# timsainb/noisereduce

Hardware: AMD Instinct MI355X
Metric: Msamples/s reduce_noise (48 kHz mono, n_fft=1024) (higher is better)
Workload: dtype f32

## Files before the change

### include/mi355gate_debug.h

```cpp
#ifndef MI355GATE_DEBUG_H
#define MI355GATE_DEBUG_H

#include "mi355gate.h"

#ifdef __cplusplus
extern "C" {
#endif

SG_API int sg_debug_dims(const sg_handle* h, int64_t dims[3]);
SG_API int sg_debug_range(const sg_handle* h, int64_t range[2]);
SG_API int sg_debug_counter(sg_handle* h, int32_t which, int64_t* value, void* stream);
SG_API int sg_debug_fetch(sg_handle* h, int32_t what, void* host, int64_t bytes, void* stream);

SG_API int sg_debug_clip_thresholds(sg_handle* h, double* host, int32_t n_noise, int32_t n_bins, void* stream);
SG_API int sg_debug_clip_batches(const sg_handle* h, int64_t* value);
SG_API int sg_debug_rows_batches(const sg_handle* h, int64_t* value);
#define SG_BWD_ROW 1
#define SG_BWD_FAST 2
#define SG_BWD_REG 3
#define SG_BWD_OLA 4
#define SG_BWD_ROWS 5
SG_API int sg_debug_backward_route(const sg_handle* h, int64_t* value);

#define SG_OPT_FORCE_UNFUSED 1
#define SG_OPT_FORCE_F64_DECIDE 3
#define SG_OPT_FORCE_NOSEAM 4
#define SG_OPT_FORCE_NOLEAN 5
#define SG_OPT_FORCE_SPLIT 6
#define SG_OPT_INJECT_HANDOFF_FAULT 7
#define SG_OPT_FORCE_NOROWGATE 10
#define SG_OPT_ROWGATE_TAP 11
#define SG_OPT_ROWGATE_SHAPE 12
#define SG_OPT_FLOOR_TEST 13
#define SG_OPT_TILE_ORDER 15
#define SG_OPT_EXACT_MATERIALISED 16
#define SG_OPT_FORCE_NOFAST 2

#define SG_STAGE_CHANNEL_MEAN 0
#define SG_STAGE_STFT_POWER 1
#define SG_STAGE_COLMAX 2
#define SG_STAGE_COLSTATS 3
#define SG_STAGE_DECIDE 4
#define SG_STAGE_STFT_MAG 5
#define SG_STAGE_NONSTAT_MASK 6
#define SG_STAGE_SMOOTH 7
#define SG_STAGE_APPLY_ISTFT 8
#define SG_STAGE_OLA 9
#define SG_STAGE_NOISE_STATS 10
#define SG_STAGE_PREP 11
// ... 29 lines not shown
```

### noisereduce_amd/_ffi.py

```python
import contextlib
import ctypes
import os
import threading
import weakref
from ctypes import (POINTER, Structure, byref, c_char_p, c_double, c_int, c_int32,
                    c_int64, c_void_p)

import numpy as np
import torch

_HERE = os.path.dirname(os.path.abspath(__file__))
LIB_PATH = os.path.join(_HERE, "libmi355gate.so")

SG_F32, SG_F64, SG_I16, SG_I32 = 0, 1, 2, 3
SG_VARIANT_S, SG_VARIANT_T = 0, 1
SG_E_INVALID, SG_E_UNSUPPORTED, SG_E_HIP, SG_E_NOMEM, SG_E_STATE, SG_E_HANDOFF = -1, -2, -3, -4, -5, -6
SG_N_STAGES = 27
SG_N_STAGES_ALL = 29
SG_OPT_FORCE_F64_DECIDE = 3
SG_OPT_FORCE_NOSEAM = 4
SG_OPT_FORCE_NOLEAN = 5
SG_OPT_FORCE_SPLIT = 6
SG_OPT_INJECT_HANDOFF_FAULT = 7
SG_OPT_FAST_INTEGER = 8
SG_OPT_FORCE_EXACT = 9
SG_OPT_FORCE_NOROWGATE = 10
SG_OPT_ROWGATE_TAP = 11
SG_OPT_ROWGATE_SHAPE = 12
SG_OPT_FLOOR_TEST = 13
SG_OPT_TILE_ORDER = 15
SG_OPT_EXACT_MATERIALISED = 16
SG_OPT_FORCE_UNFUSED = 1
SG_OPT_FORCE_NOFAST = 2
SG_BWD_ROW, SG_BWD_FAST, SG_BWD_REG, SG_BWD_OLA, SG_BWD_ROWS = 1, 2, 3, 4, 5

_TORCH_DTYPES = {torch.float32: SG_F32, torch.float64: SG_F64, torch.int16: SG_I16,
                 torch.int32: SG_I32}


class HandoffTimeout(RuntimeError):
    """SG_E_HANDOFF: a bounded inter-workgroup wait of a fused kernel timed out (the device was preempted for
    about a second); the outputs of the calls enqueued since the last check are invalid and must be re-run."""


class SgParams(Structure):
    _fields_ = [
# ... 64 lines not shown
                                  c_int64, c_int64, c_int64, c_int64, c_int32, c_int64, c_int64,
                                  c_void_p]),
    "sg_filter_padded": (c_int, [c_void_p, c_void_p, c_int, c_void_p, c_int, c_int64, c_int64,
                                 c_int64, c_int64, c_void_p]),
    "sg_process_batch": (c_int, [c_void_p, c_void_p, c_int, c_int64, c_int64, c_int64, c_void_p,
                                 c_int64, c_int64, c_int64, c_void_p, c_int, c_int64, c_void_p,
                                 c_void_p]),
    "sg_process_batch_backward": (c_int, [c_void_p, c_void_p, c_int, c_int64, c_int64, c_int64,
                                          c_void_p, c_void_p, c_int64, c_void_p]),
    "sg_process_rows": (c_int, [c_void_p, c_void_p, c_int, c_int64, c_int64, c_int64, c_void_p, c_void_p, c_int64,
                                c_int64, c_int64, c_void_p, c_void_p, c_int, c_int64, c_void_p, c_void_p]),
    "sg_process_rows_backward": (c_int, [c_void_p, c_void_p, c_int, c_int64, c_int64, c_int64, c_void_p, c_void_p,
                                         c_void_p, c_int64, c_void_p]),
    "sg_debug_rows_batches": (c_int, [c_void_p, POINTER(c_int64)]),
    "sg_debug_backward_route": (c_int, [c_void_p, POINTER(c_int64)]),
    "sg_stft": (c_int, [c_void_p, c_void_p, c_int, c_int64, c_int64, c_int64, c_void_p, c_void_p]),
    "sg_clips_workspace_bytes": (c_int, [c_void_p, c_void_p, c_int32, c_void_p, c_int64, POINTER(c_int64)]),
    "sg_process_clips": (c_int, [c_void_p, c_void_p, c_int, c_void_p, c_int, c_void_p, c_int32, c_void_p, c_int64,
                                 c_void_p, c_int, c_int64, c_void_p]),
    "sg_debug_clip_thresholds": (c_int, [c_void_p, POINTER(c_double), c_int32, c_int32, c_void_p]),
    "sg_debug_clip_batches": (c_int, [c_void_p, POINTER(c_int64)]),
    "sg_stream_create": (c_int, [c_void_p, c_int32, c_int32, c_int64, POINTER(c_void_p)]),
    "sg_stream_destroy": (c_int, [c_void_p]),
    "sg_stream_set_threshold": (c_int, [c_void_p, c_void_p, c_int32, c_void_p, c_int32, c_void_p]),
    "sg_stream_push": (c_int, [c_void_p, c_void_p, c_int, c_void_p, c_int, c_void_p, c_int32, c_void_p]),
    "sg_stream_reset": (c_int, [c_void_p, c_void_p, c_int32, c_void_p]),
    "sg_stream_emitted": (c_int, [c_void_p, c_int64, POINTER(c_int64)]),
    "sg_stream_counters": (c_int, [c_void_p, c_int32, POINTER(c_int64), POINTER(c_int64)]),
    "sg_stream_create_nonstationary": (c_int, [c_void_p, c_int32, c_int32, c_int64, c_int32, POINTER(c_void_p)]),
    "sg_stream_state_bytes": (c_int, [c_void_p, c_int32, c_int32, c_int64, c_int32, POINTER(c_int64)]),
# ... 651 lines not shown
```

### noisereduce_amd/csrc/api.hip

```cpp
#include <hip/hip_runtime.h>
#include <dlfcn.h>

#include <algorithm>
#include <cmath>
#include <cstdarg>
#include <cstdio>
#include <cstring>
#include <map>
#include <mutex>
#include <string>
#include <vector>

#include "../../include/mi355gate_debug.h"
#pragma clang fp contract(on)
#include "kernels.hpp"
#include "fused.hpp"
#include "czt.hpp"
#include "mixed.hpp"
#include "onepass.hpp"
#include "rowgate.hpp"
#include "rowbwd.hpp"
#include "fast512.hpp"
#include "onepass512.hpp"
#include "fast256.hpp"
// ... 90 lines not shown
  unsigned inject_fault = 0;
  unsigned lose_now = 0;
  unsigned ticket_base = 0;
  unsigned epoch = 0;
  bool fast_integer = false;
  bool force_exact = false;
  bool exact_materialised = false;
  DevBuf norm64;
  unsigned need_era = 0;
  DevBuf xP, xraw, xM, xtmp, xseg;
  bool force_split = false;
  int rowgate_mode = 0;
  int64_t n_floor_lazy = 0, n_floor_apriori = 0;
  int tile_order = 0;
  int n_cu = 0;
  int floor_test = 0;
  int rg_shape = 16;
  bool rg_tap = false;
  bool dbg_rg = false;
  int dbg_bwd_route = 0;
  DevBuf rg_count;
  bool dbg_xbits = false;
  int dbg_trows = 16, dbg_tstep = 16, dbg_twords = 0, dbg_txw = 9;
  int64_t dbg_tf0 = 0;
  int dbg_ntt = 0;
  int big_M = 0;
  int big_czt = 0;
  DevBuf big_twM, big_tw2, big_ch, big_bh, big_W, big_W2;
  int czt_M = 0;
  bool mr_ok = false;
// ... 1815 lines not shown
}

static int handoff_next_epoch(sg_handle* h, hipStream_t st) {
  if (++h->epoch == 0) {
    if (h->xbits.p) HIPCHK(h, hipMemsetAsync(h->xbits.p, 0, h->xbits.bytes, st));
    if (h->xpart.p) HIPCHK(h, hipMemsetAsync(h->xpart.p, 0, h->xpart.bytes, st));
    h->epoch = 1;
    if (h->err_host) h->err_host[1] = 0u;
  }
  return SG_OK;
}

static int handoff_prepare(sg_handle* h, hipStream_t st) {
  {
    bool fresh = false;
    int rc = ensure_zeroed(h, h->xticket, 64, st, &fresh);
    if (rc) return rc;
    if (fresh) h->ticket_base = 0;
  }
  if (!h->err_host) {
    HIPCHK(h, hipHostMalloc((void**)&h->err_host, 64, hipHostMallocMapped));
    *h->err_host = 0u;
    h->err_host[1] = 0u;
    HIPCHK(h, hipHostGetDevicePointer((void**)&h->err_dev, h->err_host, 0));
  }
  if (*h->err_host != 0u) {
    const unsigned e = *h->err_host;
    *h->err_host = 0u;
    FAIL(h, SG_E_HANDOFF, "a tile hand-off of an EARLIER call on this handle timed out (code %u): that call's output "
                          "is invalid (call sg_check_errors after a call to learn about it in time)", e);
  }
  h->lose_now = 0;
  if (h->inject_fault) {
// ... 157 lines not shown
  P.ticket = (unsigned*)h->xticket.p;
  P.epoch = h->epoch;
  P.err = h->err_dev;
  P.ticket_base = h->ticket_base;
  const bool persist = lazy && h->tile_order == 0 && !(h->lose_now & 3u) && ub * ntt >= 2;
  if (persist && h->n_cu == 0) {
    int dev = 0, cus = 0;
    HIPCHK(h, hipGetDevice(&dev));
    HIPCHK(h, hipDeviceGetAttribute(&cus, hipDeviceAttributeMultiprocessorCount, dev));
    h->n_cu = cus > 0 ? cus : 256;
  }
  static const int pg_per_cu = [] { const char* e = getenv("SG_ONEPASS_WG_PER_CU"); int v = e ? atoi(e) : 3; return v >= 1 && v <= 3 ? v : 3; }();
#if OP_MAX_ITERS == 1
  const unsigned pgrid = persist ? (unsigned)(ub * ntt) : 0u;
#else
  const unsigned pgrid = persist ? (unsigned)std::min<int64_t>(ub * ntt, (int64_t)pg_per_cu * h->n_cu) : 0u;
#endif
  P.total_tiles = (unsigned)(ub * ntt);
  if (h->tile_order == 1) P.ticket_base = 0xffffffffu;
  else h->ticket_base += (unsigned)(ub * ntt) + (OP_MAX_ITERS == 1 ? 0u : pgrid);
  P.nf = h->p.n_grad_freq; P.nt = h->p.n_grad_time;
  P.prop = (float)h->p.prop_decrease;
  P.inv_ktot = 1.0f / (float)h->ktot;
#if OP_WHO
  if (!g_who_dev) HIPCHK(h, hipMalloc((void**)&g_who_dev, 4096 * 16));
  HIPCHK(h, hipMemsetAsync(g_who_dev, 0, 4096 * 16, st));
  P.who = g_who_dev;
#endif
#if OP_TRACE
  {
    static unsigned* tr = nullptr;
    static size_t tr_slots = 0;
    const size_t slots = (size_t)ub * ntt * 4;
    if (!tr || tr_slots < slots) {
      HIPCHK(h, hipMalloc((void**)&tr, slots * 64));
// ... 24 lines not shown
          fprintf(stderr, "[OP_TRACE] completed waves %.0f; average shader cycles per wave and phase:", w);
          double tot = 0;
          for (int k = 0; k < 14; ++k) { fprintf(stderr, " %d:%.0f", k, sum[k] / (w > 0 ? w : 1)); tot += sum[k] / (w > 0 ? w : 1); }
          fprintf(stderr, "  sum %.0f  longest wave %.0f\n", tot, mx);
        });
      }
    }
    HIPCHK(h, hipMemsetAsync(tr, 0, slots * 64, st));
    P.trace = tr;
    g_trace_dev = tr; g_trace_tiles = (size_t)ub * ntt; g_trace_ntt = (int)ntt;
  }
#endif
  {
    ProfScope ps(h, SG_STAGE_ONEPASS, st);
    const size_t lds = (size_t)(fast::FN + WAVES * fast::WAVE_CX_H) * sizeof(fast::cf) + (1024 + T2_FLOATS) * sizeof(float) +
                       256 * 8 + 514 * 8 + 192 * 8 + 32 + (prop ? 528 : 0);
    auto go = [&](auto kern) -> hipError_t {
      hipError_t e = set_lds(reinterpret_cast<const void*>(kern), lds);
      if (e != hipSuccess) return e;
      hipLaunchKernelGGL(kern, dim3(persist ? pgrid : (unsigned)(ub * ntt)), dim3(WAVES * 64), lds, st, P);
      return hipGetLastError();
    };
    if (persist && prop) HIPCHK(h, go(fast::k_gate_onepass<WAVES, true, false, false, true>));
    else if (persist) HIPCHK(h, go(fast::k_gate_onepass<WAVES, false, false, false, true>));
    else if (h->lose_now & 3u) HIPCHK(h, go(fast::k_gate_onepass<WAVES, false, true>));
    else if (prop) HIPCHK(h, go(fast::k_gate_onepass<WAVES, true>));
    else HIPCHK(h, go(fast::k_gate_onepass<WAVES, false>));
  }
  if (lazy) {
    ProfScope ps(h, SG_STAGE_STFT_MAX, st);
    const int wpr = (g.F + 63) / 64;
    HIPCHK(h, launch_bits_any<0>(h, vx, g, ub, tc,
                             (unsigned long long*)h->pmax.p, (unsigned long long*)h->bits.p, wpr, st));
    if ((rc = handoff_next_epoch(h, st))) return rc;
    P.epoch = h->epoch;
    P.ticket = (unsigned*)h->xticket.p + 8;
    P.ticket_base = 0;
    const size_t lds = (size_t)(fast::FN + WAVES * fast::WAVE_CX_H) * sizeof(fast::cf) + (1024 + T2_FLOATS) * sizeof(float) +
                       256 * 8 + 514 * 8 + 192 * 8 + 32 + (prop ? 528 : 0);
    auto redo = [&](auto kern) -> hipError_t {
      hipError_t e = set_lds(reinterpret_cast<const void*>(kern), lds);
      if (e != hipSuccess) return e;
      hipLaunchKernelGGL(kern, dim3((unsigned)(ub * ntt)), dim3(WAVES * 64), lds, st, P);
      return hipGetLastError();
    };
    if (prop) HIPCHK(h, redo(fast::k_gate_onepass<WAVES, true, false, true>));
    else HIPCHK(h, redo(fast::k_gate_onepass<WAVES, false, false, true>));
    HIPCHK(h, hipGetLastError());
  }
  h->dbg_xbits = true;
  h->dbg_trows = 16; h->dbg_tstep = 16; h->dbg_twords = fast::OP_TILE_WORDS; h->dbg_txw = fast::OP_XW;
  h->dbg_tf0 = A.h_begin - 3;
  h->dbg_ntt = (int)ntt;
  h->dbg_db = std::max<int64_t>(0, A.h_begin - 3 - NF);
// ... 819 lines not shown
    case SG_OPT_FORCE_NOROWGATE:
      if (value < 0 || value > 2) FAIL(h, SG_E_INVALID, "SG_OPT_FORCE_NOROWGATE: 0 (auto), 1 (never) or 2 (always)");
      h->rowgate_mode = (int)value;
      return SG_OK;
    case SG_OPT_ROWGATE_TAP: h->rg_tap = value != 0; return SG_OK;
    case SG_OPT_ROWGATE_SHAPE:
      if (value != 8 && value != 16) FAIL(h, SG_E_INVALID, "SG_OPT_ROWGATE_SHAPE: 8 or 16 waves");
      h->rg_shape = (int)value;
      return SG_OK;
    case SG_OPT_INJECT_HANDOFF_FAULT: h->inject_fault = (unsigned)value & 63u; return SG_OK;
    case SG_OPT_TILE_ORDER:
      if (value < 0 || value > 2) FAIL(h, SG_E_INVALID, "SG_OPT_TILE_ORDER: 0 (persistent workgroups), 1 (block index) or 2 (one ticket per workgroup)");
      h->tile_order = (int)value;
      return SG_OK;
    case SG_OPT_EXACT_MATERIALISED: h->exact_materialised = value != 0; return SG_OK;
    case SG_OPT_FLOOR_TEST:
      if (value < 0 || value > 2) FAIL(h, SG_E_INVALID, "SG_OPT_FLOOR_TEST: 0 (predicted), 1 (a priori) or 2 (in the gate kernel)");
      h->floor_test = (int)value;
      return SG_OK;
  }
  FAIL(h, SG_E_INVALID, "sg_set_option: unknown option %d", option);
}

extern "C" int sg_get_option(const sg_handle* h, int32_t option, int64_t* value) {
  if (!h || !value) return SG_E_INVALID;
  switch (option) {
    case SG_OPT_FORCE_UNFUSED: *value = h->force_unfused; return SG_OK;
    case SG_OPT_FORCE_NOFAST: *value = h->force_nofast; return SG_OK;
    case SG_OPT_FORCE_F64_DECIDE: *value = h->force_f64_decide; return SG_OK;
    case SG_OPT_FORCE_NOSEAM: *value = h->force_noseam; return SG_OK;
    case SG_OPT_FORCE_NOLEAN: *value = h->force_nolean; return SG_OK;
    case SG_OPT_FORCE_SPLIT: *value = h->force_split; return SG_OK;
    case SG_OPT_FAST_INTEGER: *value = h->fast_integer; return SG_OK;
    case SG_OPT_FORCE_EXACT: *value = h->force_exact; return SG_OK;
    case SG_OPT_FORCE_NOROWGATE: *value = h->rowgate_mode; return SG_OK;
    case SG_OPT_ROWGATE_TAP: *value = h->rg_tap; return SG_OK;
    case SG_OPT_ROWGATE_SHAPE: *value = h->rg_shape; return SG_OK;
    case SG_OPT_INJECT_HANDOFF_FAULT: *value = h->inject_fault; return SG_OK;
    case SG_OPT_TILE_ORDER: *value = h->tile_order; return SG_OK;
    case SG_OPT_EXACT_MATERIALISED: *value = h->exact_materialised; return SG_OK;
    case SG_OPT_FLOOR_TEST: *value = h->floor_test; return SG_OK;
  }
  return SG_E_INVALID;
}

extern "C" int sg_profile_enable(sg_handle* h, int32_t on) {
  if (!h) return SG_E_INVALID;
  h->prof_on = on != 0;
  return SG_OK;
}

extern "C" int sg_profile_select(sg_handle* h, int64_t stage_mask) {
  if (!h) return SG_E_INVALID;
  h->prof_mask = stage_mask == 0 ? ~0ull : (uint64_t)stage_mask;
  return SG_OK;
// ... 51 lines not shown
  if (!h || !dims) return SG_E_INVALID;
  dims[0] = h->dbg_units; dims[1] = h->dbg_T; dims[2] = h->FS;
  return SG_OK;
}

extern "C" int sg_debug_range(const sg_handle* h, int64_t range[2]) {
  if (!h || !range) return SG_E_INVALID;
  range[0] = h->dbg_db; range[1] = h->dbg_de;
  return SG_OK;
}

extern "C" int sg_debug_counter(sg_handle* h, int32_t which, int64_t* value, void* stream) {
  if (!h || !value) return SG_E_INVALID;
  if (which == 1 || which == 2) {
    *value = which == 1 ? h->n_floor_lazy : h->n_floor_apriori;
    return SG_OK;
  }
  if (which == 3) {
    HIPCHK(h, hipStreamSynchronize((hipStream_t)stream));
    *value = h->err_host ? (int64_t)h->err_host[1] : 0;
    return SG_OK;
  }
#if OP_TRACE
  if (which == 8) {
    HIPCHK(h, hipStreamSynchronize((hipStream_t)stream));
    std::vector<unsigned> t(g_trace_tiles * 64);
    HIPCHK(h, hipMemcpy(t.data(), g_trace_dev, t.size() * 4, hipMemcpyDeviceToHost));
    int64_t bad = 0;
    auto last_phase = [&](size_t tk, int w) { int lp = -1; for (int k = 0; k < 14; ++k) if (t[(tk * 4 + w) * 16 + k]) lp = k; return lp; };
    for (size_t tk = 0; tk < g_trace_tiles; ++tk) {
// ... 189 lines not shown
  if (h->p.variant != SG_VARIANT_T) FAIL(h, SG_E_INVALID, "sg_process_rows_backward is a variant-T entry point");
  if (!grad_out_dev || !grad_x_dev || !mask_dev || B < 1 || (dtype != SG_F32 && dtype != SG_F64) || gx_stride < L ||
      L < 2 * (int64_t)h->W)
    FAIL(h, SG_E_INVALID, "sg_process_rows_backward: bad argument");
  h->dbg_bwd_route = SG_BWD_ROWS;
  return sg::rw_backward(&h->rw, rg_ctx(h), grad_out_dev, dtype, B, L, go_stride, lengths, mask_dev, grad_x_dev, gx_stride,
                         rw_budget(h), (hipStream_t)stream, &h->err);
}

extern "C" int sg_debug_rows_batches(const sg_handle* h, int64_t* value) {
  if (!h || !value) return SG_E_INVALID;
  *value = sg::rw_last_batches(h->rw);
  return SG_OK;
}

extern "C" int sg_debug_backward_route(const sg_handle* h, int64_t* value) {
  if (!h || !value) return SG_E_INVALID;
  *value = h->dbg_bwd_route;
  return SG_OK;
}

struct sg_stream_bank {
  sg_handle* h;
  sg::StBank* b;
};

static int stream_create(sg_handle* h, const sg_stream_desc& d, const char* who, sg_stream_bank** out) {
  if (h->p.variant != SG_VARIANT_S) FAIL(h, SG_E_INVALID, "%s is a variant-S entry point", who);
  sg::StBank* b = nullptr;
  const sg::StAdaptive ad{d.forget, d.learn_frames};
// ... 162 lines not shown
```

### noisereduce_amd/csrc/onepass.hpp

```cpp
#pragma once
#include "fastpath.hpp"

namespace sg {
namespace fast {

constexpr int OP_XW = 9;
constexpr int OP_TILE_WORDS = 16 * OP_XW * 2;
constexpr int OP_MAX_NT = 16;
constexpr int OP_KP = 528;
constexpr int OP_TAB_WIN = 0, OP_TAB_WSQ = 4096, OP_TAB_INVN = 8192, OP_TAB_TW512 = 9216, OP_TAB_TW1024 = 13312,
              OP_TAB_WIN64 = 17408, OP_TAB_TW64 = 25600, OP_TAB_MCONST = 33792, OP_TAB_EXP8 = 35328, OP_TAB_BYTES = 37376;

#ifndef OP_LATE_ARGS
#define OP_LATE_ARGS 1
#endif
#ifndef OP_TRACE
#define OP_TRACE 0
#endif
#ifndef OP_ARGCHECK
#define OP_ARGCHECK 0
#endif
#ifndef OP_TILECOUNT
#define OP_TILECOUNT 0
#endif
// ... 36 lines not shown
  int dtype_exact;
  const char* tab;
  ThreshConsts tc;
  double mag_scale, top_db;
  unsigned long long* xbits;
  unsigned* ticket;
  unsigned ticket_base;
  unsigned epoch;
  unsigned* err;
  int nf, nt;
  float prop, inv_ktot;
  unsigned long long* part2;
  unsigned* alim;
  int scan_q;
  unsigned total_tiles;
#if OP_TRACE
  unsigned* trace;
#endif
#if OP_WHO
  unsigned* who;
#endif
};

#if OP_LATE_ARGS
#define OP_XARG(type, member) (*(const __attribute__((address_space(4))) type*)(kp4 + __builtin_offsetof(OnePassArgs, member)))
#else
#define OP_XARG(type, member) (P.member)
#endif
__device__ __forceinline__ double op_exact_power(const OnePassArgs& P, int64_t row, int64_t chunk, int64_t t, int f,
                                                 int lane) {
// ... 32 lines not shown
__device__ __forceinline__ float4 op_ldg4(const float* p) {
  const op_v4f v = *(const OP_G4 op_v4f*)p;
  return make_float4(v[0], v[1], v[2], v[3]);
}
__device__ __forceinline__ void op_stg4(float* p, float4 a) {
  const op_v4f v = {a.x, a.y, a.z, a.w};
  *(OP_G4 op_v4f*)p = v;
}
__device__ __forceinline__ unsigned op_draw_ticket_late(unsigned long long p64) {
#if OP_WAIT_SITES & 1
  asm volatile("" : "+v"(p64));
  return __hip_atomic_fetch_add((__attribute__((address_space(1))) unsigned*)p64, 1u, __ATOMIC_RELAXED, __HIP_MEMORY_SCOPE_AGENT);
#else
  return atomicAdd((unsigned*)(uintptr_t)p64, 1u);
#endif
}

__device__ __forceinline__ void op_err_or(unsigned* p, unsigned bits) {
  __HIP_ATOMIC_BACKWARD_COMPAT_MEMORY {
    __hip_atomic_fetch_or((__attribute__((address_space(1))) unsigned*)p, bits, __ATOMIC_RELAXED, __HIP_MEMORY_SCOPE_SYSTEM);
  }
}

template <int M>
__device__ __forceinline__ int op_xor_lanes(int v) {
  static_assert(M > 0 && M < 32, "within a half-wave");
  return __builtin_amdgcn_ds_swizzle(v, (M << 10) | 0x1f);
}

#ifndef OP_ABLATE
// ... 25 lines not shown
#endif
constexpr unsigned OP_SEAM_NONE = 0xffffffffu;
template <int WAVES, bool PROP, bool LOSE = false, bool REDO = false, bool PERSIST = false>
__global__ __launch_bounds__(WAVES * 64, OP_OCC) void k_gate_onepass(OnePassArgs Pk) {
  static_assert(WAVES == 4, "tile = 16 frames");
  static_assert(!PERSIST || (!LOSE && !REDO), "the persistent loop is the lazy first launch only");
  extern __shared__ __attribute__((aligned(16))) char smem[];
  cf* tw512 = reinterpret_cast<cf*>(smem);
  cf* regions = tw512 + FN;
  float* swin = reinterpret_cast<float*>(regions + WAVES * WAVE_CX_H);
  float* s_t2 = swin + 1024;
  unsigned long long* s_exp = reinterpret_cast<unsigned long long*>(s_t2 + T2_FLOATS);
  double* s_t2d = reinterpret_cast<double*>(s_exp + 256);
  unsigned long long* s_mc = reinterpret_cast<unsigned long long*>(s_t2d + 514);
  unsigned* s_misc = reinterpret_cast<unsigned*>(s_mc + 192);
  unsigned char* s_ef = reinterpret_cast<unsigned char*>(s_misc + 8);
  constexpr int NF = 4 * WAVES;
  constexpr int SPAN = (NF - 1) * 256 + 1024, XPITCH = 288;
  static_assert((SPAN / 256) * XPITCH <= WAVES * WAVE_CX_H * 2, "span must fit the exchange slices");
  constexpr int NQ = SPAN / 256;
  static_assert(SPAN % 256 == 0 && WAVES * 64 == 256, "one sample per thread and row");
  constexpr int SCAN_REG = 5;

  if (REDO && Pk.alim[1] != Pk.tc.need_tag) return;
#if OP_LATE_START_US
  if (PERSIST && (blockIdx.x % 5u) == 1u) {
    const unsigned long long t0_ = wall_clock64();
    while ((long long)(wall_clock64() - t0_) < (long long)OP_LATE_START_US * 100 * (1 + (blockIdx.x % 7u))) __builtin_amdgcn_s_sleep(8);
  }
#endif
  double t2pre[3];
// ... 3 lines not shown
    static_assert(FN == 2 * WAVES * 64 && WAVES * 64 == 256, "one pass of the prologue loads per thread");
    const cf tw_a = reinterpret_cast<const cf*>(Pk.tab + OP_TAB_TW512)[(tid >> 4) * (tid & 15)];
    const cf tw_b = reinterpret_cast<const cf*>(Pk.tab + OP_TAB_TW512)[((tid + 256) >> 4) * (tid & 15)];
    const float4 w4 = reinterpret_cast<const float4*>(Pk.tab + OP_TAB_WIN)[tid];
    const unsigned long long e8 = reinterpret_cast<const unsigned long long*>(Pk.tab + OP_TAB_EXP8)[tid];
    const unsigned long long mc8 = reinterpret_cast<const unsigned long long*>(Pk.tab + OP_TAB_MCONST)[min(tid, 191)];
    t2pre[0] = Pk.tc.T2[perm_inv(tid)];
    t2pre[1] = Pk.tc.T2[perm_inv(tid + 256)];
    t2pre[2] = Pk.tc.T2[perm_inv(512)];
    if (!REDO && Pk.alim != nullptr) {
      int z = 2 + min(lane & 15, OP_ALIM_BLOCKS - 1);
      asm volatile("" : "+v"(z));
      alim_v = Pk.alim[z];
    }
    if (tid == 0) {
      s_misc[PERSIST ? 4 : 0] = Pk.ticket_base == 0xffffffffu ? blockIdx.x : atomicAdd(Pk.ticket, 1u) - Pk.ticket_base;
      s_misc[1] = 0u;
      if (PERSIST) s_misc[0] = OP_SEAM_NONE;
    }
    tw512[tid] = tw_a;
    tw512[tid + 256] = tw_b;
    reinterpret_cast<float4*>(swin)[tid] = w4;
    s_exp[tid] = e8;
    if (tid < 192) s_mc[tid] = mc8;
    if constexpr (PROP) {
      for (int f = tid; f <= 512; f += WAVES * 64) {
        const int lo = max(-Pk.nf, -f), hi = min(Pk.nf, 512 - f);
        int sum = 0;
        for (int a = lo; a <= hi; ++a) sum += Pk.nf + 1 - (a < 0 ? -a : a);
        s_ef[f] = (unsigned char)sum;
      }
// ... 526 lines not shown
    }
  }

  OP_STAMP(5);
#if OP_LATE_ARGS
  typedef const __attribute__((address_space(4))) char* op_kpm_t;
  op_kpm_t kpm = (op_kpm_t)__builtin_amdgcn_kernarg_segment_ptr();
  asm volatile("" : "+s"(kpm));
#define OP_MARG(type, member) (*(const __attribute__((address_space(4))) type*)(kpm + __builtin_offsetof(OnePassArgs, member)))
  const unsigned m_ticket = (unsigned)__builtin_amdgcn_readfirstlane((int)s_misc[tk_slot]);
  const unsigned m_ntt = (unsigned)(OP_MARG(int, A.n_tiles) + 2);
  const int64_t m_u = m_ticket / m_ntt;
  const int m_jt = (int)(m_ticket % m_ntt) - 1;
#else
#define OP_MARG(type, member) (P.member)
  const unsigned m_ntt = (unsigned)ntt;
  const int64_t m_u = u;
  const int m_jt = jt;
#endif
  unsigned long long* const m_xbits = (unsigned long long*)(uintptr_t)OP_MARG(unsigned long long, xbits);
  const unsigned m_epoch = OP_MARG(unsigned, epoch);
  unsigned* const m_err = (unsigned*)(uintptr_t)OP_MARG(unsigned long long, err);
  const char* const m_tab = (const char*)(uintptr_t)OP_MARG(unsigned long long, tab);
  const float m_kscale = OP_MARG(float, A.kscale);
  const int m_nt = OP_MARG(int, nt);
  [[maybe_unused]] const float m_inv_ktot = OP_MARG(float, inv_ktot), m_prop = OP_MARG(float, prop);
  unsigned long long* xb_mine = m_xbits + ((size_t)m_u * m_ntt + (m_jt + 1)) * OP_TILE_WORDS;
  if (c < OP_XW) {
    const op_v4u gr = {(unsigned)myword, m_epoch, (unsigned)(myword >> 32), m_epoch};
    op_st16_sc1(&xb_mine[((4 * wave + g) * OP_XW + c) * 2], gr);
  }
  [[maybe_unused]] unsigned pend_halo = OP_SEAM_NONE;
  if constexpr (DEFER) {
    if (halo_tile) pend_halo = (unsigned)__builtin_amdgcn_readfirstlane((int)s_misc[0]);
  }
  __syncthreads();
  if (halo_tile) {
    if constexpr (DEFER) {
      seam_close(pend_halo, tid);
      if (tid == 0) s_misc[0] = OP_SEAM_NONE;
    }
    if constexpr (PERSIST) {
#if OP_MAX_ITERS == 1 || OP_DRAW_TOP
      if (tid == 0) s_misc[tk_slot ^ 1u] = 0xffffffffu;
#else
      if (tid == 0) s_misc[tk_slot ^ 1u] = op_draw_ticket_late(OP_MARG(unsigned long long, ticket)) - OP_MARG(unsigned, ticket_base);
#endif
      pf = false;
#pragma unroll
      for (int k = 0; k < NQ; ++k) q[k] = 0.f;
#pragma unroll
      for (int k = 0; k < SCAN_REG; ++k) sc[k] = 0.f;
    }
    OP_DONE;
  }
  OP_STAMP(6);

  constexpr int WP = OP_XW + 2;
  constexpr int WPB = WP * 8;
  constexpr int SLICE_B = WAVE_CX_H * 8;
  char* rbytes = reinterpret_cast<char*>(regions);
// ... 46 lines not shown
        op_err_or(m_err, 1u);
#if OP_WHO
        if (atomicAdd_system(m_err + 14, 1u) == 0u) { m_err[8] = m_ticket; m_err[9] = (unsigned)i; m_err[10] = gr[1]; m_err[11] = m_epoch; }
#endif
        s_misc[1] = 1u;
        break;
      }
      OP_POLL_SLEEP(spin);
      gr = op_ld16_sc1(src);
    }
    wb[(side ? m_nt + NF + rr : rr) * WP + 1 + w] = (unsigned long long)gr[0] | ((unsigned long long)gr[2] << 32);
  }
  __syncthreads();
  OP_STAMP(8);
  [[maybe_unused]] unsigned nx_raw = 0u;
  if constexpr (PERSIST) {
#if OP_MAX_ITERS == 1 || OP_DRAW_TOP
    if (tid == 0) nx_raw = 0xffffffffu + OP_MARG(unsigned, ticket_base);
#else
    if (tid == 0) nx_raw = op_draw_ticket_late(OP_MARG(unsigned long long, ticket));
#endif
  }
  {
    const unsigned char* rp1 = wbb + r1 * WPB + 7 + q4;
    const unsigned char* rp2 = wbb + r2 * WPB + 7 + q4;
#pragma unroll
    for (int nb = 0; nb < 9; ++nb) {
      const int b = wave + 4 * nb;
      if (b < 33) {
        const long a1 = (long)s_exp[rp1[2 * b]];
        const op_v4i h1 = __builtin_amdgcn_mfma_i32_16x16x32_i8(a1, Bf, zero4, 0, 0, 0);
        const unsigned p1 = (unsigned)h1[0] | ((unsigned)h1[1] << 8) | ((unsigned)h1[2] << 16) | ((unsigned)h1[3] << 24);
        const long bt1 = (long)(((unsigned long long)p1 << 32) | (unsigned long long)hown[nb]);
        op_v4i d = __builtin_amdgcn_mfma_i32_16x16x32_i8(At1, bt1, zero4, 0, 0, 0);
        if (three) {
          const long a2 = (long)s_exp[rp2[2 * b]];
          const op_v4i h2 = __builtin_amdgcn_mfma_i32_16x16x32_i8(a2, Bf, zero4, 0, 0, 0);
          const unsigned p2 = (unsigned)h2[0] | ((unsigned)h2[1] << 8) | ((unsigned)h2[2] << 16) | ((unsigned)h2[3] << 24);
          d = __builtin_amdgcn_mfma_i32_16x16x32_i8(At2, (long)(unsigned long long)p2, d, 0, 0, 0);
        }
        unsigned short* kd = reinterpret_cast<unsigned short*>(rbytes + q4 * (SLICE_B + 64)) + 16 * b + j16;
        kd[0] = (unsigned short)d[0];
        kd[OP_KP] = (unsigned short)d[1];
        kd[2 * OP_KP] = (unsigned short)d[2];
        kd[3 * OP_KP] = (unsigned short)d[3];
      }
    }
  }
#if !OP_TK_LATE
  if constexpr (PERSIST) {
    if (tid == 0) s_misc[tk_slot ^ 1u] = nx_raw - OP_MARG(unsigned, ticket_base);
#if OP_WHO
    if (tid == 0) {
      unsigned* w_ = (unsigned*)(uintptr_t)OP_MARG(unsigned long long, who);
      const unsigned nx_ = nx_raw - OP_MARG(unsigned, ticket_base);
      if (nx_ < 4096u) { w_[nx_ * 4] = (blockIdx.x + 1u) | (iter << 16); w_[nx_ * 4 + 1] = m_ticket; }
      if (m_ticket < 4096u) w_[m_ticket * 4 + 3] = 1u;
    }
#endif
  }
#endif
  __syncthreads();
  OP_STAMP(9);

  const unsigned short* kt = reinterpret_cast<const unsigned short*>(rbytes + wave * (SLICE_B + 64));
  const unsigned short* krow = kt + g * OP_KP;
  const unsigned short* k_lo = krow + (c == 0 ? 0 : c);
  const unsigned short* k_hi = krow + (c == 0 ? 0 : 32 - c);
  float tt = 0.f;
  if constexpr (PROP) {
// ... 62 lines not shown
    for (int i = 1; i < 8; ++i) v[i] = pa[i];
    v[8] = sel(z8, pa[8]);
#pragma unroll
    for (int i = 9; i < 16; ++i) v[i] = sel(pb[16 - i], pa[i]);
#pragma unroll
    for (int i = 16; i < 24; ++i) v[i] = sel(pa[i - 8], pb[31 - i]);
#pragma unroll
    for (int i = 24; i < 31; ++i) v[i] = sel(pb[39 - i], pb[31 - i]);
    v[31] = sel(pb[8], pb[0]);
  }
#endif
  wave_lds_sync();
  OP_STAMP(10);
#if OP_TK_LATE
  if constexpr (PERSIST) {
    if (tid == 0) *(volatile unsigned*)&s_misc[tk_slot ^ 1u] = nx_raw - OP_MARG(unsigned, ticket_base);
  }
#endif

  {
    int zi = 0, ci = c;
    asm volatile("" : "+v"(zi), "+v"(ci));
    fft512_inv_half(v, fb + zi, tw512 + zi, ci);
  }
  OP_STAMP(11);
  float4 n4;
  auto load_n4 = [&]() { n4 = op_ldg4(&reinterpret_cast<const float*>(m_tab + OP_TAB_INVN)[(tid & 63) * 4]); };
  if constexpr (PERSIST) load_n4();
  auto prefetch_next = [&]() {
    const OnePassArgs& Pn = *late_args<OnePassArgs>();
#if OP_TK_LATE
// ... 297 lines not shown
```

Before: 108,000.

## Split persistent onepass ticket counter into three heads over tile ranges

Result: no change. 109,000 (median of 6 runs) (+0.9%).

```diff
diff --git a/include/mi355gate_debug.h b/include/mi355gate_debug.h
--- a/include/mi355gate_debug.h
+++ b/include/mi355gate_debug.h
@@ -21,6 +21,7 @@
 #define SG_BWD_OLA 4
 #define SG_BWD_ROWS 5
 SG_API int sg_debug_backward_route(const sg_handle* h, int64_t* value);
+SG_API int sg_debug_onepass_heads(int64_t units, int64_t tiles_per_unit, int64_t workgroups, int64_t lo[4]);
 
 #define SG_OPT_FORCE_UNFUSED 1
 #define SG_OPT_FORCE_F64_DECIDE 3
@@ -33,6 +34,10 @@
 #define SG_OPT_ROWGATE_SHAPE 12
 #define SG_OPT_FLOOR_TEST 13
 #define SG_OPT_TILE_ORDER 15
+#define SG_OPT_ONEPASS_HEADS 17
+#define SG_OPT_ONEPASS_DELAY_NS 18
+#define SG_OPT_ONEPASS_GROUP_BY 19
+#define SG_OPT_ONEPASS_GRID 20
 #define SG_OPT_EXACT_MATERIALISED 16
 #define SG_OPT_FORCE_NOFAST 2
 
diff --git a/noisereduce_amd/_ffi.py b/noisereduce_amd/_ffi.py
--- a/noisereduce_amd/_ffi.py
+++ b/noisereduce_amd/_ffi.py
@@ -30,6 +30,10 @@
 SG_OPT_FLOOR_TEST = 13
 SG_OPT_TILE_ORDER = 15
 SG_OPT_EXACT_MATERIALISED = 16
+SG_OPT_ONEPASS_HEADS = 17
+SG_OPT_ONEPASS_DELAY_NS = 18
+SG_OPT_ONEPASS_GROUP_BY = 19
+SG_OPT_ONEPASS_GRID = 20
 SG_OPT_FORCE_UNFUSED = 1
 SG_OPT_FORCE_NOFAST = 2
 SG_BWD_ROW, SG_BWD_FAST, SG_BWD_REG, SG_BWD_OLA, SG_BWD_ROWS = 1, 2, 3, 4, 5
@@ -124,6 +128,7 @@
                                          c_void_p, c_int64, c_void_p]),
     "sg_debug_rows_batches": (c_int, [c_void_p, POINTER(c_int64)]),
     "sg_debug_backward_route": (c_int, [c_void_p, POINTER(c_int64)]),
+    "sg_debug_onepass_heads": (c_int, [c_int64, c_int64, c_int64, POINTER(c_int64)]),
     "sg_stft": (c_int, [c_void_p, c_void_p, c_int, c_int64, c_int64, c_int64, c_void_p, c_void_p]),
     "sg_clips_workspace_bytes": (c_int, [c_void_p, c_void_p, c_int32, c_void_p, c_int64, POINTER(c_int64)]),
     "sg_process_clips": (c_int, [c_void_p, c_void_p, c_int, c_void_p, c_int, c_void_p, c_int32, c_void_p, c_int64,
diff --git a/noisereduce_amd/csrc/api.hip b/noisereduce_amd/csrc/api.hip
--- a/noisereduce_amd/csrc/api.hip
+++ b/noisereduce_amd/csrc/api.hip
@@ -128,6 +128,12 @@
   int64_t n_floor_lazy = 0, n_floor_apriori = 0;
   int tile_order = 0;
   int n_cu = 0;
+  unsigned head_base[2] = {0, 0};
+  int op_heads = 0;
+  int op_delay_ns = OP_HEAD_DELAY_NS;
+  int op_group_by = OP_GROUP_BY;
+  int dbg_heads = 0;
+  int op_grid = 0;
   int floor_test = 0;
   int rg_shape = 16;
   bool rg_tap = false;
@@ -1973,9 +1979,9 @@
 static int handoff_prepare(sg_handle* h, hipStream_t st) {
   {
     bool fresh = false;
-    int rc = ensure_zeroed(h, h->xticket, 64, st, &fresh);
+    int rc = ensure_zeroed(h, h->xticket, (2 * fast::OP_HEAD_STRIDE + 16) * 4, st, &fresh);
     if (rc) return rc;
-    if (fresh) h->ticket_base = 0;
+    if (fresh) h->ticket_base = h->head_base[0] = h->head_base[1] = 0;
   }
   if (!h->err_host) {
     HIPCHK(h, hipHostMalloc((void**)&h->err_host, 64, hipHostMallocMapped));
@@ -2163,11 +2169,36 @@
 #if OP_MAX_ITERS == 1
   const unsigned pgrid = persist ? (unsigned)(ub * ntt) : 0u;
 #else
-  const unsigned pgrid = persist ? (unsigned)std::min<int64_t>(ub * ntt, (int64_t)pg_per_cu * h->n_cu) : 0u;
+  const unsigned pgrid = persist ? (unsigned)std::min<int64_t>(std::min<int64_t>(ub * ntt, (int64_t)pg_per_cu * h->n_cu),
+                                                               h->op_grid > 0 ? std::max(2, h->op_grid) : INT64_MAX) : 0u;
 #endif
   P.total_tiles = (unsigned)(ub * ntt);
+  P.n_heads = 1;
+  P.head_lo[0] = 0; P.head_lo[1] = P.head_lo[2] = P.head_lo[3] = P.total_tiles;
+  P.head_base[0] = P.ticket_base; P.head_base[1] = h->head_base[0]; P.head_base[2] = h->head_base[1];
+  P.head_delay = 0; P.group_by = 0;
+  if (persist && !(OP_MAX_ITERS == 1) && h->op_heads != 1) {
+    int64_t lo[4];
+    unsigned in_group[3] = {0, 0, 0};
+    const unsigned gb = (unsigned)h->op_group_by;
+    for (unsigned b = 0; b < pgrid; ++b) ++in_group[gb == 1u ? (b / 8u) % 3u : (unsigned)((uint64_t)b * 3u / pgrid)];
+    const bool alone_ok = ub % 3 == 0 && std::min(in_group[0], std::min(in_group[1], in_group[2])) >= 2u;
+    if (fast::onepass_heads(ub, ntt, pgrid, lo) == 3 && alone_ok) {
+      P.n_heads = 3;
+      for (int i = 0; i < 4; ++i) P.head_lo[i] = (unsigned)lo[i];
+      P.head_delay = (unsigned)(h->op_delay_ns / 10);
+      P.group_by = gb;
+    }
+  }
+  h->dbg_heads = persist ? (int)P.n_heads : 0;
   if (h->tile_order == 1) P.ticket_base = 0xffffffffu;
-  else h->ticket_base += (unsigned)(ub * ntt) + (OP_MAX_ITERS == 1 ? 0u : pgrid);
+  else if (P.n_heads == 3) {
+    unsigned over[3] = {0, 0, 0};
+    for (unsigned b = 0; b < pgrid; ++b) ++over[P.group_by == 1u ? (b / 8u) % 3u : (unsigned)((uint64_t)b * 3u / pgrid)];
+    h->ticket_base += (P.head_lo[1] - P.head_lo[0]) + over[0];
+    h->head_base[0] += (P.head_lo[2] - P.head_lo[1]) + over[1];
+    h->head_base[1] += (P.head_lo[3] - P.head_lo[2]) + over[2];
+  } else h->ticket_base += (unsigned)(ub * ntt) + (OP_MAX_ITERS == 1 ? 0u : pgrid);
   P.nf = h->p.n_grad_freq; P.nt = h->p.n_grad_time;
   P.prop = (float)h->p.prop_decrease;
   P.inv_ktot = 1.0f / (float)h->ktot;
@@ -2222,7 +2253,7 @@
   {
     ProfScope ps(h, SG_STAGE_ONEPASS, st);
     const size_t lds = (size_t)(fast::FN + WAVES * fast::WAVE_CX_H) * sizeof(fast::cf) + (1024 + T2_FLOATS) * sizeof(float) +
-                       256 * 8 + 514 * 8 + 192 * 8 + 32 + (prop ? 528 : 0);
+                       256 * 8 + 514 * 8 + 192 * 8 + 64 + (prop ? 528 : 0);
     auto go = [&](auto kern) -> hipError_t {
       hipError_t e = set_lds(reinterpret_cast<const void*>(kern), lds);
       if (e != hipSuccess) return e;
@@ -2245,7 +2276,7 @@
     P.ticket = (unsigned*)h->xticket.p + 8;
     P.ticket_base = 0;
     const size_t lds = (size_t)(fast::FN + WAVES * fast::WAVE_CX_H) * sizeof(fast::cf) + (1024 + T2_FLOATS) * sizeof(float) +
-                       256 * 8 + 514 * 8 + 192 * 8 + 32 + (prop ? 528 : 0);
+                       256 * 8 + 514 * 8 + 192 * 8 + 64 + (prop ? 528 : 0);
     auto redo = [&](auto kern) -> hipError_t {
       hipError_t e = set_lds(reinterpret_cast<const void*>(kern), lds);
       if (e != hipSuccess) return e;
@@ -3095,6 +3126,22 @@
       h->tile_order = (int)value;
       return SG_OK;
     case SG_OPT_EXACT_MATERIALISED: h->exact_materialised = value != 0; return SG_OK;
+    case SG_OPT_ONEPASS_HEADS:
+      if (value != 0 && value != 1) FAIL(h, SG_E_INVALID, "SG_OPT_ONEPASS_HEADS: 0 (three heads where the launch is large enough) or 1 (one head)");
+      h->op_heads = (int)value;
+      return SG_OK;
+    case SG_OPT_ONEPASS_DELAY_NS:
+      if (value < 0 || value > 100000) FAIL(h, SG_E_INVALID, "SG_OPT_ONEPASS_DELAY_NS: 0 .. 100000");
+      h->op_delay_ns = (int)value;
+      return SG_OK;
+    case SG_OPT_ONEPASS_GROUP_BY:
+      if (value < 0 || value > 1) FAIL(h, SG_E_INVALID, "SG_OPT_ONEPASS_GROUP_BY: 0 (block index, thirds of the grid) or 1 (block index / 8, modulo 3)");
+      h->op_group_by = (int)value;
+      return SG_OK;
+    case SG_OPT_ONEPASS_GRID:
+      if (value < 0 || value > 0x7fffffff) FAIL(h, SG_E_INVALID, "SG_OPT_ONEPASS_GRID: 0 (three workgroups per compute unit) or a number of workgroups");
+      h->op_grid = (int)value;
+      return SG_OK;
     case SG_OPT_FLOOR_TEST:
       if (value < 0 || value > 2) FAIL(h, SG_E_INVALID, "SG_OPT_FLOOR_TEST: 0 (predicted), 1 (a priori) or 2 (in the gate kernel)");
       h->floor_test = (int)value;
@@ -3120,6 +3167,10 @@
     case SG_OPT_INJECT_HANDOFF_FAULT: *value = h->inject_fault; return SG_OK;
     case SG_OPT_TILE_ORDER: *value = h->tile_order; return SG_OK;
     case SG_OPT_EXACT_MATERIALISED: *value = h->exact_materialised; return SG_OK;
+    case SG_OPT_ONEPASS_HEADS: *value = h->op_heads; return SG_OK;
+    case SG_OPT_ONEPASS_DELAY_NS: *value = h->op_delay_ns; return SG_OK;
+    case SG_OPT_ONEPASS_GROUP_BY: *value = h->op_group_by; return SG_OK;
+    case SG_OPT_ONEPASS_GRID: *value = h->op_grid; return SG_OK;
     case SG_OPT_FLOOR_TEST: *value = h->floor_test; return SG_OK;
   }
   return SG_E_INVALID;
@@ -3201,6 +3252,10 @@
   if (!h || !value) return SG_E_INVALID;
   if (which == 1 || which == 2) {
     *value = which == 1 ? h->n_floor_lazy : h->n_floor_apriori;
+    return SG_OK;
+  }
+  if (which == 17) {
+    *value = h->dbg_heads;
     return SG_OK;
   }
   if (which == 3) {
@@ -3420,6 +3475,11 @@
   return SG_OK;
 }
 
+extern "C" int sg_debug_onepass_heads(int64_t units, int64_t tiles_per_unit, int64_t workgroups, int64_t lo[4]) {
+  if (!lo || units < 0 || tiles_per_unit < 0 || workgroups < 0) return SG_E_INVALID;
+  return fast::onepass_heads(units, tiles_per_unit, workgroups, lo);
+}
+
 extern "C" int sg_debug_backward_route(const sg_handle* h, int64_t* value) {
   if (!h || !value) return SG_E_INVALID;
   *value = h->dbg_bwd_route;
diff --git a/noisereduce_amd/csrc/onepass.hpp b/noisereduce_amd/csrc/onepass.hpp
--- a/noisereduce_amd/csrc/onepass.hpp
+++ b/noisereduce_amd/csrc/onepass.hpp
@@ -74,6 +74,11 @@
   unsigned* alim;
   int scan_q;
   unsigned total_tiles;
+  unsigned head_lo[4];
+  unsigned head_base[3];
+  unsigned n_heads;
+  unsigned head_delay;
+  unsigned group_by;
 #if OP_TRACE
   unsigned* trace;
 #endif
@@ -136,6 +141,32 @@
 #else
   return atomicAdd((unsigned*)(uintptr_t)p64, 1u);
 #endif
+}
+
+constexpr unsigned OP_HEAD_STRIDE = 32;
+constexpr int OP_ST_HEAD = 8;
+#ifndef OP_HEAD_DELAY_NS
+#define OP_HEAD_DELAY_NS 0
+#endif
+#ifndef OP_GROUP_BY
+#define OP_GROUP_BY 1
+#endif
+inline int onepass_heads(int64_t units, int64_t ntt, int64_t workgroups, int64_t lo[4]) {
+  const int64_t per_group = (workgroups + 2) / 3;
+  lo[0] = 0;
+  for (int g = 1; g <= 3; ++g) lo[g] = units * g / 3 * ntt;
+  const int64_t least = std::min(lo[1] - lo[0], std::min(lo[2] - lo[1], lo[3] - lo[2]));
+  if (units >= 3 && workgroups >= 6 && least >= 2 * per_group) return 3;
+  lo[1] = lo[2] = lo[3] = units * ntt;
+  return 1;
+}
+#define OP_HARG(type, member) (*(const __attribute__((address_space(4))) type*)(kh + __builtin_offsetof(OnePassArgs, member)))
+__device__ __forceinline__ unsigned op_head_next(const unsigned* st) {
+  const __attribute__((address_space(4))) char* kh = (const __attribute__((address_space(4))) char*)__builtin_amdgcn_kernarg_segment_ptr();
+  asm volatile("" : "+s"(kh));
+  const uint4 hd = *reinterpret_cast<const uint4*>(st);
+  const unsigned tk = op_draw_ticket_late(OP_HARG(unsigned long long, ticket) + hd.w) - hd.y;
+  return tk < hd.z ? tk : 0xffffffffu;
 }
 
 __device__ __forceinline__ void op_err_or(unsigned* p, unsigned bits) {
@@ -191,7 +222,7 @@
   double* s_t2d = reinterpret_cast<double*>(s_exp + 256);
   unsigned long long* s_mc = reinterpret_cast<unsigned long long*>(s_t2d + 514);
   unsigned* s_misc = reinterpret_cast<unsigned*>(s_mc + 192);
-  unsigned char* s_ef = reinterpret_cast<unsigned char*>(s_misc + 8);
+  unsigned char* s_ef = reinterpret_cast<unsigned char*>(s_misc + 16);
   constexpr int NF = 4 * WAVES;
   constexpr int SPAN = (NF - 1) * 256 + 1024, XPITCH = 288;
   static_assert((SPAN / 256) * XPITCH <= WAVES * WAVE_CX_H * 2, "span must fit the exchange slices");
@@ -225,7 +256,23 @@
       alim_v = Pk.alim[z];
     }
     if (tid == 0) {
-      s_misc[PERSIST ? 4 : 0] = Pk.ticket_base == 0xffffffffu ? blockIdx.x : atomicAdd(Pk.ticket, 1u) - Pk.ticket_base;
+      if constexpr (PERSIST) {
+        unsigned grp = 0u;
+        if (Pk.n_heads == 3u) {
+          grp = Pk.group_by == 1u ? (blockIdx.x / 8u) % 3u : blockIdx.x * 3u / gridDim.x;
+          const unsigned long long t0_ = wall_clock64();
+          while ((unsigned long long)(wall_clock64() - t0_) < (unsigned long long)grp * Pk.head_delay) __builtin_amdgcn_s_sleep(8);
+        }
+        const unsigned lo_ = Pk.head_lo[grp], adj_ = Pk.head_base[grp] - lo_, hi_ = Pk.head_lo[grp + 1u];
+        s_misc[OP_ST_HEAD] = grp;
+        s_misc[OP_ST_HEAD + 1] = adj_;
+        s_misc[OP_ST_HEAD + 2] = hi_;
+        s_misc[OP_ST_HEAD + 3] = grp * OP_HEAD_STRIDE * 4u;
+        const unsigned tk_ = atomicAdd(Pk.ticket + grp * OP_HEAD_STRIDE, 1u) - adj_;
+        s_misc[4] = tk_ < hi_ ? tk_ : 0xffffffffu;
+      } else {
+        s_misc[0] = Pk.ticket_base == 0xffffffffu ? blockIdx.x : atomicAdd(Pk.ticket, 1u) - Pk.ticket_base;
+      }
       s_misc[1] = 0u;
       if (PERSIST) s_misc[0] = OP_SEAM_NONE;
     }
@@ -782,6 +829,7 @@
   const int m_jt = (int)(m_ticket % m_ntt) - 1;
 #else
 #define OP_MARG(type, member) (P.member)
+  [[maybe_unused]] const unsigned m_ticket = ticket;
   const unsigned m_ntt = (unsigned)ntt;
   const int64_t m_u = u;
   const int m_jt = jt;
@@ -812,7 +860,7 @@
 #if OP_MAX_ITERS == 1 || OP_DRAW_TOP
       if (tid == 0) s_misc[tk_slot ^ 1u] = 0xffffffffu;
 #else
-      if (tid == 0) s_misc[tk_slot ^ 1u] = op_draw_ticket_late(OP_MARG(unsigned long long, ticket)) - OP_MARG(unsigned, ticket_base);
+      if (tid == 0) s_misc[tk_slot ^ 1u] = op_head_next(&s_misc[OP_ST_HEAD]);
 #endif
       pf = false;
 #pragma unroll
@@ -889,11 +937,21 @@
   __syncthreads();
   OP_STAMP(8);
   [[maybe_unused]] unsigned nx_raw = 0u;
+  [[maybe_unused]] uint4 hd_st = make_uint4(0u, 0u, 0u, 0u);
+  auto nx_ticket = [&]() -> unsigned {
+#if OP_MAX_ITERS == 1 || OP_DRAW_TOP
+    return nx_raw - OP_MARG(unsigned, ticket_base);
+#else
+    const unsigned tk_ = nx_raw - hd_st.y;
+    return tk_ < hd_st.z ? tk_ : 0xffffffffu;
+#endif
+  };
   if constexpr (PERSIST) {
 #if OP_MAX_ITERS == 1 || OP_DRAW_TOP
     if (tid == 0) nx_raw = 0xffffffffu + OP_MARG(unsigned, ticket_base);
 #else
-    if (tid == 0) nx_raw = op_draw_ticket_late(OP_MARG(unsigned long long, ticket));
+    hd_st = *reinterpret_cast<const uint4*>(&s_misc[OP_ST_HEAD]);
+    if (tid == 0) nx_raw = op_draw_ticket_late(OP_MARG(unsigned long long, ticket) + hd_st.w);
 #endif
   }
   {
@@ -924,11 +982,12 @@
   }
 #if !OP_TK_LATE
   if constexpr (PERSIST) {
-    if (tid == 0) s_misc[tk_slot ^ 1u] = nx_raw - OP_MARG(unsigned, ticket_base);
+    [[maybe_unused]] unsigned nx_tk_ = 0u;
+    if (tid == 0) s_misc[tk_slot ^ 1u] = nx_tk_ = nx_ticket();
 #if OP_WHO
     if (tid == 0) {
       unsigned* w_ = (unsigned*)(uintptr_t)OP_MARG(unsigned long long, who);
-      const unsigned nx_ = nx_raw - OP_MARG(unsigned, ticket_base);
+      const unsigned nx_ = nx_tk_;
       if (nx_ < 4096u) { w_[nx_ * 4] = (blockIdx.x + 1u) | (iter << 16); w_[nx_ * 4 + 1] = m_ticket; }
       if (m_ticket < 4096u) w_[m_ticket * 4 + 3] = 1u;
     }
@@ -1021,7 +1080,7 @@
   OP_STAMP(10);
 #if OP_TK_LATE
   if constexpr (PERSIST) {
-    if (tid == 0) *(volatile unsigned*)&s_misc[tk_slot ^ 1u] = nx_raw - OP_MARG(unsigned, ticket_base);
+    if (tid == 0) *(volatile unsigned*)&s_misc[tk_slot ^ 1u] = nx_ticket();
   }
 #endif
 
```
